# google-research/frame-interpolation

Hardware: AMD Instinct MI355X
Metric: interpolated frames/sec @1080p (higher is better)
Workload: dtype f32; 1 GPU; 1080p_2x2: 1920x1080 pair, align 64, block_shape [2, 2] -> 4 tile(s) of 960x576 in one batch, film_net published config, seeded synthetic weights, t=0.5; parallelism=1 independent GPU(s), weights RCCL-broadcast once, exec=direct launches, two lanes, lanes=1

## Files before the change

frame-interpolation_amd/csrc/conv_wino2d_impl.h:

```cpp
#pragma once
#include "conv_common.h"

enum { W2D_F_SQ = 128,
       W2D_F_XEPI = 8,
       W2D_DBG_TIME = 8192 };


template <bool SQ> struct W2dSlotTable { unsigned v[24 * 64]; };
template <bool SQ> constexpr W2dSlotTable<SQ> w2d_make_slot_table() {
  constexpr int QW = SQ ? 4 : 8, TH = SQ ? 16 : 8, HR = TH + 2, PW = 4 * QW + 2;
  constexpr int CO4 = (PW + 3) / 4, MO4 = 4 * CO4, RP4 = 4 * MO4 + (SQ ? 2 : 4);
  W2dSlotTable<SQ> t{};
  for (int sl = 0; sl < 24 * 64; ++sl) {
    const int r = sl / RP4, rem = sl % RP4, m = rem / MO4, rr = rem % MO4, c = rr / CO4, k = rr % CO4, px = 4 * k + m;
    const bool ok = r < HR && rem < 4 * MO4 && px < PW;
    t.v[sl] = ok ? ((unsigned)r << 24 | (unsigned)px << 8 | (unsigned)c << 4) : 0xFFFFFFFFu;
  }
  return t;
}
template <bool SQ> __device__ const W2dSlotTable<SQ> w2d_slot_table = w2d_make_slot_table<SQ>();

template <int BN, int FLAGS, int NS_ = 3>
__global__ __launch_bounds__(4 * (BN / 32) * 64, (BN == 32) ? 2 : 1) void conv_wino2d_kernel(ConvParams p) {
  constexpr bool SQ = (FLAGS & W2D_F_SQ) != 0;
  constexpr int QW = SQ ? 4 : 8, TH = SQ ? 16 : 8, HR = TH + 2, PXW = 4 * QW, PW = PXW + 2;
  static_assert(QW * (TH / 2) == 32, "32 units per tile");
  constexpr int NG = BN / 32, NW = 4 * NG;
  constexpr int CO4 = (PW + 3) / 4, MO4 = 4 * CO4, RP4 = 4 * MO4 + (SQ ? 2 : 4);
  constexpr int NREQ = 24;
  constexpr int STAGE4 = NREQ * 64;
  constexpr int NS = NS_;
  static_assert(NS == 2 || NS == 3, "stages");
  constexpr int IPW = NREQ / NW;
  static_assert(NREQ % NW == 0, "requests per wave");
  static_assert(HR * RP4 <= STAGE4, "stage size");
  constexpr bool XE = (FLAGS & W2D_F_XEPI) != 0;
  constexpr unsigned OOB = 0xFFFFFFFFu;

  extern __shared__ __attribute__((aligned(1024))) float smem[];

  const int t = threadIdx.x;
  const int lane = t & 63;
  const int wv = __builtin_amdgcn_readfirstlane(t >> 6);
  const int l31 = lane & 31, half = lane >> 5;
  const int mu = wv & 3, ng = wv >> 2;

  unsigned long long tm0 = 0, tm1 = 0, tm2 = 0, tmA = 0, tmB = 0, tmC = 0, tmW = 0, tmE1 = 0, tmE2 = 0, tmE3 = 0;
  unsigned long long rt0 = 0;
  if constexpr ((FLAGS & W2D_DBG_TIME) != 0) { rt0 = __builtin_amdgcn_s_memrealtime(); tm0 = __builtin_readcyclecounter(); }

  int aH = p.H, aW = p.W, aNB = p.NB, aCtot = p.Ctot, aKsplit = p.ksplit, aNseg = p.nseg, aUnused = p.unused_chain;
// ... 298 lines not shown
    for (int r = 0; r < 16; ++r) {
      const float m0 = acc[0][r], m1 = acc[1][r], m2 = acc[2][r], m3 = acc[3][r], m4 = acc[4][r], m5 = acc[5][r];
      const float s34 = m3 + m4, d34 = m3 - m4, d12 = m1 - m2, s12 = m1 + m2;
      o[0][r] = ((m0 + m1) + m2) + s34;
      o[1][r] = __builtin_fmaf(2.f, d34, d12);
      o[2][r] = __builtin_fmaf(4.f, s34, s12);
      o[3][r] = d12 + __builtin_fmaf(8.f, d34, m5);
    }
    bf4* const xb = reinterpret_cast<bf4*>(smem);
    constexpr int XB4 = NG * 4 * 256;
    static_assert(2 * XB4 <= NS * STAGE4, "exchange buffers");
    const int widx = (ng * 4 + mu) * 256 + l31 * 8;
    const int rng = t >> 8, run = (t >> 3) & 31, rcg = t & 7;
    const int ridx = rng * 1024 + run * 8 + (rcg ^ (run & 7));
    const int nrd = n0 + rng * 32 + rcg * 4;
    const bool rawsum = XE && ksp > 1;
    const bool has_pw = XE && p.pw_out != nullptr;
    float b0 = 0.f, b1 = 0.f, b2 = 0.f, b3 = 0.f;
    if (!rawsum) { const float* const bp = p.bias + nrd; b0 = bp[0]; b1 = bp[1]; b2 = bp[2]; b3 = bp[3]; }
    const int oy = y0 + 2 * (run / QW), ox = x0 + 4 * (run % QW);
    const int ostr = rawsum ? p.Cout : p.ostride;
    const float slope = (p.leaky && !rawsum) ? 0.2f : 1.f;
    const int dyo = 2 * (run / QW), dxo = 4 * (run % QW), nth = rng * 32 + rcg * 4;
    const int cpix = (img * p.H + y0) * p.W + x0;
    float* obase = p.out;
    if (rawsum) { asm volatile(""); obase = p.part + (size_t)blockIdx.z * p.M * p.Cout; }
    float* const ocorner = obase + ((long long)cpix * ostr + n0);
    float* const orow = ocorner + (__umul24(__umul24(dyo, p.W) + dxo, ostr) + nth);
    float* pool_base = nullptr;
    if (XE && p.pool_out) {
      asm volatile("");
      const int ppix = (img * (p.H >> 1) + (y0 >> 1)) * (p.W >> 1) + (x0 >> 1);
      pool_base = p.pool_out + ((long long)ppix * p.pool_ostride + n0) + (__umul24(__umul24(dyo >> 1, p.W >> 1) + (dxo >> 1), p.pool_ostride) + nth);
    }
    constexpr int PWS = 68;
    float* const pwt = smem + 2 * XB4 * 4;
    float* const pww = pwt + TH * PXW * PWS;
    if (has_pw && t < 256) pww[t] = (t & 3) < p.pw_cout ? p.pw_w[(t >> 2) * p.pw_cout + (t & 3)] : 0.f;
    bf4 k0 = {0.f, 0.f, 0.f, 0.f}, k1 = {0.f, 0.f, 0.f, 0.f};
    auto write_round = [&](int jx, bf4* xw) {
  #pragma unroll
      for (int g = 0; g < 4; ++g) {
        bf4 v;
        v[0] = o[jx][4 * g]; v[1] = o[jx][4 * g + 1]; v[2] = o[jx][4 * g + 2]; v[3] = o[jx][4 * g + 3];
        xw[widx + ((2 * g + half) ^ (l31 & 7))] = v;
      }
    };
  #pragma unroll
    for (int jx = 0; jx < 4; ++jx) {
      bf4* const xw = xb + (jx & 1) * XB4;
      write_round(jx, xw);
      __syncthreads();
      if constexpr ((FLAGS & W2D_DBG_TIME) != 0) { if (jx == 0) tmE2 = __builtin_readcyclecounter(); if (jx == 3) tmE3 = __builtin_readcyclecounter(); }
// ... 18 lines not shown
          if (jx & 1) {
            bf4 pv;
  #pragma unroll
            for (int c = 0; c < 4; ++c) pv[c] = (((k0[c] + r0[c]) + k1[c]) + r1[c]) * 0.25f;
            if (oy < p.H && ox + jx < p.W) *reinterpret_cast<bf4*>(pool_base + (size_t)(jx >> 1) * p.pool_ostride) = pv;
          } else {
            k0 = r0; k1 = r1;
          }
        }
      } else {
        float* const tr = pwt + ((2 * (run / QW)) * PXW + 4 * (run % QW) + jx) * PWS + rng * 32 + rcg * 4;
        *reinterpret_cast<bf4*>(tr) = r0;
        *reinterpret_cast<bf4*>(tr + PXW * PWS) = r1;
      }
    }
    if (has_pw) {
      __syncthreads();
      if (t < TH * PXW) {
        const int y = y0 + t / PXW, x = x0 + (t % PXW);
        float a[4] = {0.f, 0.f, 0.f, 0.f};
        const bf4* row = reinterpret_cast<const bf4*>(pwt + t * PWS);
        const bf4* wq = reinterpret_cast<const bf4*>(pww);
  #pragma unroll 4
        for (int c4 = 0; c4 < 16; ++c4) {
          const bf4 v = row[c4];
  #pragma unroll
          for (int k = 0; k < 4; ++k) {
            const bf4 w = wq[c4 * 4 + k];
  #pragma unroll
            for (int j = 0; j < 4; ++j) a[j] = __builtin_fmaf(v[k], w[j], a[j]);
          }
// ... 25 lines not shown
  if constexpr ((FLAGS & W2D_DBG_TIME) != 0) {
    const unsigned long long tm3 = __builtin_readcyclecounter();
    if (t == 0) {
      unsigned long long* o8 = reinterpret_cast<unsigned long long*>(p.part) + (size_t)(blockIdx.y * gridDim.x + blockIdx.x) * 16;
      o8[0] = tm0; o8[1] = tm1; o8[2] = tm2; o8[3] = tm3; o8[4] = tmA; o8[5] = tmB; o8[6] = tmC; o8[7] = tmW;
      o8[8] = rt0; o8[9] = __builtin_amdgcn_s_memrealtime();
      o8[10] = (unsigned long long)__builtin_amdgcn_s_getreg((31 << 11) | 4) | ((unsigned long long)__builtin_amdgcn_s_getreg((31 << 11) | 20) << 32);
      o8[11] = tmE1; o8[12] = tmE2; o8[13] = tmE3; o8[14] = tmK; o8[15] = tmT;
    }
  }
}

template <int BN, int FLAGS, int NS = 3>
hipError_t conv_wino2d_launch(const ConvParams& p, hipStream_t s) {
  if (!(FLAGS & W2D_F_XEPI) && (p.ksplit > 1 || p.pool_out || p.pw_out)) return hipErrorInvalidValue;
  const size_t lds = p.pw_out ? (size_t)2 * (BN / 32) * 16 * 1024 + 256 * 68 * 4 + 1024 : (size_t)NS * 24 * 1024;
  constexpr int NT = 4 * (BN / 32) * 64;
  if (p.ksize != 3 || p.Ctot % 16 || p.Cout % BN) return hipErrorInvalidValue;
  if (p.ksplit > 1 && (!p.part || (reinterpret_cast<uintptr_t>(p.part) & 15) || p.Cout % 4 || p.pool_out || p.pw_out || p.ksplit > p.Ctot / 16)) return hipErrorInvalidValue;
  if (p.pw_out) {
    if (BN != 64 || p.Cout != 64 || p.pool_out || p.pw_cout < 1 || p.pw_cout > 4) return hipErrorInvalidValue;
  } else if (p.ostride % 4 || (reinterpret_cast<uintptr_t>(p.out) & 15)) return hipErrorInvalidValue;
  if (p.pool_out && ((p.H | p.W) & 1 || p.pool_ostride % 4 || (reinterpret_cast<uintptr_t>(p.pool_out) & 15))) return hipErrorInvalidValue;
  {
    long long nimg = p.NB;
    for (int i = 0; i < p.nseg; ++i) nimg = std::max<long long>(nimg, (long long)p.seg[i].bmod);
    if ((nimg + 1) * p.H * p.W >= (1ll << 31)) return hipErrorInvalidValue;
  }
  if (p.W <= 0 || p.H <= 0 || p.W >= (1 << 20) || p.ostride >= (1 << 22) || p.pool_ostride >= (1 << 22) || p.Cout >= (1 << 22) ||
      (long long)8 * p.W * (p.ostride > p.Cout ? p.ostride : p.Cout) >= (1ll << 31)) return hipErrorInvalidValue;
  for (int i = 0; i < p.nseg; ++i)
    if ((long long)p.W * p.seg[i].stride * 4 >= (1ll << 24) || p.seg[i].C % 16 || p.seg[i].stride % 4 || p.seg[i].stride <= 0 || p.seg[i].stride >= (1 << 22) || p.seg[i].up || (reinterpret_cast<uintptr_t>(p.seg[i].ptr) & 15)) return hipErrorInvalidValue;
  constexpr bool SQ = (FLAGS & W2D_F_SQ) != 0;
  const int ntx = SQ ? (p.W + 15) / 16 : (p.W + 31) / 32, nty = SQ ? (p.H + 15) / 16 : (p.H + 7) / 8;
  const int ntiles = p.NB * ntx * nty;
  dim3 grid((unsigned)ntiles, p.Cout / BN, (unsigned)(p.ksplit > 1 ? p.ksplit : 1));
  ConvParams q = p;
  bool exact = true;
  q.mg_nby = conv_magic(grid.y, (unsigned long long)grid.x * grid.y, exact);
  q.mg_tpi = conv_magic((unsigned long long)ntx * nty, (unsigned long long)ntiles + 1, exact);
  q.mg_ntx = conv_magic(ntx, (unsigned long long)ntx * nty, exact);
  q.tl_ntx = ntx; q.tl_tpi = ntx * nty;
  if (!exact) return hipErrorInvalidValue;
  return conv_launch<conv_wino2d_kernel<BN, FLAGS, NS>>(grid, dim3(NT), lds, s, q, 144 * 1024);
}

template <int BN, int FLAGS, int NS = 3>
hipError_t conv_wino2d_launch_any(const ConvParams& p, hipStream_t s) {
  if (p.ksplit > 1 || p.pool_out || p.pw_out) return conv_wino2d_launch<BN, FLAGS | W2D_F_XEPI, NS>(p, s);
  return conv_wino2d_launch<BN, FLAGS, NS>(p, s);
}
```

frame-interpolation_amd/csrc/film_engine.cpp:

```cpp
#include "film_internal.h"

namespace film_internal {

thread_local std::string g_create_error;

int fail(film_t* h, int code, const char* fmt, ...) {
  char buf[1024];
  va_list ap;
  va_start(ap, fmt);
  vsnprintf(buf, sizeof buf, fmt, ap);
  va_end(ap);
  if (h) h->err = buf; else g_create_error = buf;
  return code;
}

int copy_out_string(film_t* h, const std::string& s, char* buf, int64_t cap, int64_t* needed) {
  if (needed) *needed = (int64_t)s.size() + 1;
  if (!buf || cap < (int64_t)s.size() + 1) {
    if (!buf && needed) return FILM_OK;
    return fail(h, FILM_ERR_INVALID, "buffer too small: need %lld bytes", (long long)s.size() + 1);
  }
  memcpy(buf, s.c_str(), s.size() + 1);
  return FILM_OK;
}
// ... 23 lines not shown
    {"max_batch", &film_t::opt_max_batch, NONNEG, false},
    {"host_overlap", &film_t::opt_host_overlap, BOOL, false},
    {"block_overlap_h", &film_t::opt_block_overlap_h, AS_IS, false, -1, 65535, "block_overlap_h: -1 (what the align padding of a tile holds) or 0 .. 65535 rows"},
    {"block_overlap_w", &film_t::opt_block_overlap_w, AS_IS, false, -1, 65535, "block_overlap_w: -1 (what the align padding of a tile holds) or 0 .. 65535 columns"},
    {"scene_cut", &film_t::opt_scene_cut, AS_IS, false, 0, 1000, "scene_cut: 0 (off) or 1 .. 1000 permille of the histogram distance"},
    {"tune_ms", &film_t::opt_tune_ms, NONNEG, false},
    {"splitk", &film_t::opt_splitk, BOOL, true},
    {"pack_groups", nullptr, AS_IS, false, 1, 4, "pack_groups: 1 .. 4"},
    {"fuse", &film_t::opt_fuse, LOW5, true},
    {"fold2x2", &film_t::opt_fold2x2, AS_IS, true, 0, 2, "fold2x2: 0, 1 or 2"},
    {"planar", &film_t::opt_planar, BOOL, true},
    {"winograd", &film_t::opt_wino, AS_IS, true, 0, 3, "winograd: 0, 1, 2 or 3", FAM_WINO, 2, 2,
     "winograd = 2 (F(2,3) kernel on every level) needs a library built with FILM_EXTRA_FAMILIES=1"},
    {"halo_all", &film_t::opt_halo_all, BOOL, true, 0, 0, nullptr, FAM_HALO, 1, 1, "halo_all needs a library built with FILM_EXTRA_FAMILIES=1"},
    {"lanes", &film_t::opt_lanes, AS_IS, true, 0, 3, "lanes: 0, 1, 2 or 3"},
    {"wino2d", &film_t::opt_wino2d, AS_IS, true, 0, 2, "wino2d: 0, 1 or 2"},
    {"w2d_small_px", &film_t::opt_w2d_small_px, AS_IS, true, 0, 1 << 30, "w2d_small_px: pixels per image, 0 = never"},
    {"w2d_min_px", &film_t::opt_w2d_min_px, AS_IS, true, 1, 1 << 30, "w2d_min_px: pixels per image"},
    {"w2d_splitk", &film_t::opt_w2d_splitk, AS_IS, true, 0, 16, "w2d_splitk: 0 (off), 1 (default rule) or 2..16 (A/B: the cap on levels of <= 1024 pixels)"},
    {"w2d_shape", &film_t::opt_w2d_shape, AS_IS, true, -1, W2D_SHAPES - 1, "w2d_shape: -1 (autotuned) or a Wino2dTile shape index"},
    {"fold4_shape", &film_t::opt_fold4_shape, AS_IS, true, -1, F4_4x32, "fold4_shape: -1 (autotuned) or a Fold4Tile shape index"},
    {"w43_shape", &film_t::opt_w43_shape, AS_IS, true, -1, 31, "w43_shape: -1 (autotuned) or a Wino43Tile shape index"},
    {"precision", &film_t::opt_precision, AS_IS, true, 0, 2, "precision: 0 (f32), 1 (bf16x6) or 2 (bf16x3)", FAM_SPLIT6, 1, 2,
     "precision %d (bf16 split modes) needs a library built with FILM_EXTRA_FAMILIES=1; this build runs fp32 MFMA only"},
};
constexpr bool option_rows_complete() {
  for (const OptionRow& o : kOptions)
    if ((o.lo < o.hi) != (o.refusal != nullptr) || ((o.family != FAM_BUF) != (o.family_refusal != nullptr))) return false;
  return true;
}
// ... 665 lines not shown
  fs.primed = true; fs.slot = slot; fs.plan_id = P0->id; fs.geo = tp;
  fs.hist_valid = scene_k > 0; fs.cut = cut ? 1 : 0;
  unprime.armed = false;
  return FILM_OK;
}

int film_get_tap(film_t* h, const char* name, float* dst, int64_t cap, int64_t dims[4]) {
  if (!h || !name) return FILM_ERR_INVALID;
  if (h->plan_only) return fail(h, FILM_ERR_NO_DEVICE, "plan-only handle has no device");
  Plan* P = h->last_plan;
  if (!P || !P->arena) return fail(h, FILM_ERR_STATE, "no forward has run yet");
  const int bi = P->find(name);
  if (bi < 0) return fail(h, FILM_ERR_NOTFOUND, "unknown tap '%s'", name);
  const Buffer& b = P->bufs[bi];
  for (const OpDesc& op : P->ops)
    if (op.kind == OP_CONV && op.pw_out.buf >= 0 && op.out.buf == bi)
      return fail(h, FILM_ERR_STATE, "tap '%s' is not materialised: the RGB head is fused into the layer that produces it "
                  "(film_set_option \"fuse\" without bit 16 keeps it)", name);
  if (dims) { dims[0] = b.N; dims[1] = b.H; dims[2] = b.W; dims[3] = b.C; }
  if (!dst) return FILM_OK;
  if (cap < b.size()) return fail(h, FILM_ERR_INVALID, "capacity %lld < %lld floats", (long long)cap, (long long)b.size());
  HIPCHK(h, hipSetDevice(h->device));
  HIPCHK(h, hipDeviceSynchronize());
  if (!b.planar) {
    HIPCHK(h, hipMemcpy(dst, P->arena + b.off, (size_t)b.size() * sizeof(float), hipMemcpyDeviceToHost));
    return FILM_OK;
  }
  std::vector<float> raw((size_t)b.size());
  HIPCHK(h, hipMemcpy(raw.data(), P->arena + b.off, raw.size() * sizeof(float), hipMemcpyDeviceToHost));
  const int64_t npix = (int64_t)b.N * b.H * b.W;
  const int pc[3] = {b.planar, b.planar, b.C - 2 * b.planar};
// ... 72 lines not shown
```

frame-interpolation_amd/csrc/film_exec.cpp:

```cpp
#include "film_internal.h"

namespace film_internal {
namespace {
inline const float* cptr(const float* base, const View& v) { return base + v.off; }
inline float* mptr(float* base, const View& v) { return base + v.off; }
}

hipError_t launch_op(const OpDesc& op, float* arena, const float* wts, hipStream_t s) {
  switch (op.kind) {
    case OP_CONV: {
      ConvParams p{};
      p.nseg = op.nseg;
      for (int i = 0; i < op.nseg; ++i) {
        p.seg[i].ptr = cptr(arena, op.seg[i].v);
        p.seg[i].stride = op.seg[i].v.stride;
        p.seg[i].C = op.seg[i].v.C;
        p.seg[i].boff = op.seg[i].boff; p.seg[i].bmod = op.seg[i].bmod; p.seg[i].up = op.seg[i].up;
      }
      p.ksize = op.ksize;
      p.w = wts + op.*kConvFamily[op.family].weights;
      p.bias = wts + op.b_off;
      p.out = mptr(arena, op.out); p.ostride = op.out.stride;
      p.NB = op.NB; p.H = op.H; p.W = op.W; p.Cout = op.Cout; p.Ctot = op.Ctot; p.leaky = op.leaky;
      p.M = op.NB * op.H * op.W;
      p.fold = op.fold; p.py = op.py; p.px = op.px; p.ftaps = op.ftaps;
      p.ksplit = op.ksplit; p.part = op.ksplit > 1 ? arena + op.part_off : nullptr;
      if (op.out2.buf >= 0) { p.pool_out = mptr(arena, op.out2); p.pool_ostride = op.out2.stride; }
      if (op.pw_out.buf >= 0) {
        p.pw_w = wts + op.w2_off; p.pw_bias = wts + op.b2_off; p.pw_out = mptr(arena, op.pw_out); p.pw_ostride = op.pw_out.stride; p.pw_cout = op.pw_cout;
      }
      for (int q = 0; q < 4; ++q) { p.tdy[q] = (signed char)op.tdy[q]; p.tdx[q] = (signed char)op.tdx[q]; p.fold_woff[q] = op.fold_woff[q]; }
      return film_launch_conv(p, op.tile, s);
    }
    case OP_FLOW_HEAD: {
      FlowHeadParams p{};
      p.in = cptr(arena, op.in); p.istride = op.in.stride; p.Cin = op.Ctot;
      p.w3 = wts + op.w_off; p.b3 = wts + op.b_off; p.w4 = wts + op.w2_off; p.b4 = wts + op.b2_off;
      p.out = mptr(arena, op.out); p.M = (int)op.n;
      if (op.out2.buf >= 0) { p.add = cptr(arena, op.in2); p.sum = mptr(arena, op.out2); }
      return film_launch_flow_head(p, s);
    }
    case OP_CONV_PW: {
// ... 36 lines not shown
        p.pack_b = cptr(arena, op.pack_b); p.pack_f = cptr(arena, op.pack_f);
      }
      return film_launch_warp(p, s);
    }
    case OP_PACK_FLOW: {
      PackFlowParams p{};
      p.bflow = cptr(arena, op.in); p.fflow = cptr(arena, op.in2);
      p.dst = mptr(arena, op.out); p.dstride = op.out.stride; p.npix = op.n;
      return film_launch_pack_flow(p, s);
    }
  }
  return hipErrorInvalidValue;
}

bool batch_splittable(const OpDesc& op, int nparts) {
  return op.kind == OP_CONV && op.nseg == 1 && op.seg[0].bmod == 0 && op.seg[0].boff == 0 && op.seg[0].up == 0 && op.ksplit <= 1 && op.fold == 0 &&
         op.NB >= nparts && op.NB % nparts == 0 && (op.out2.buf < 0 || (!(op.H & 1) && !(op.W & 1)));
}
OpDesc batch_part(const OpDesc& op, int part, int nparts) {
  OpDesc q = op;
  q.NB = op.NB / nparts;
  const int64_t px = (int64_t)part * q.NB * op.H * op.W;
  q.seg[0].v.off += px * op.seg[0].v.stride;
  q.out.off += px * op.out.stride;
  if (op.out2.buf >= 0) q.out2.off += (int64_t)part * q.NB * (op.H / 2) * (op.W / 2) * op.out2.stride;
  if (op.pw_out.buf >= 0) q.pw_out.off += px * op.pw_out.stride;
  return q;
}

hipError_t issue_lanes(film_t* h, Plan* P, hipStream_t main, bool capturing, const LanePipe* lp) {
  const size_t nops = P->ops.size();
// ... 100 lines not shown
```

frame-interpolation_amd/csrc/film_internal.h:

```cpp
#pragma once
#include <hip/hip_runtime.h>

#include <algorithm>
#include <atomic>
#include <cmath>
#include <cstdarg>
#include <cstdint>
#include <cstdio>
#include <cstdlib>
#include <cstring>
#include <functional>
#include <map>
#include <memory>
#include <sstream>
#include <string>
#include <thread>
#include <vector>

#include "../../include/film_hip.h"
#include "film_kernels.h"

namespace film_internal {


// ... 32 lines not shown
  ConvFamily family = FAM_BUF;
  int64_t b_off = 0;
  int64_t w2_off = 0, b2_off = 0;
  int ksplit = 1;
  int64_t part_off = 0;
  int fold = 0, py = 0, px = 0;
  int ftaps = 0; int tdy[4] = {0, 0, 0, 0}, tdx[4] = {0, 0, 0, 0};
  int64_t fold_woff[4] = {0, 0, 0, 0};
  int lane = 0;
  std::vector<int> xdeps;
  bool signal = false;
  View in, in2, out;
  View pack_b, pack_f;
  View img_in, img_out;
  View pw_out; int pw_cout = 0;
  View in3, out2;
  int NB = 0, H = 0, W = 0;
  float fscale = 1.f;
  int src_brot = 0, flow_brot = 0, misc_nb = 0;
  int64_t n = 0;
  double flops = 0;
  double bytes = 0;
};

struct LayerPack : ConvWeights {
  std::string name;
  int kh, kw, cin, cout;
  std::vector<int> perm;
  bool c3 = false;
  bool kmajor() const { return !c3 && cout % 32 == 0; }
// ... 92 lines not shown
  int opt_graph = 2;
  int opt_profile = 0, opt_autotune = 1;
  int opt_max_batch = 0;
  int opt_block_overlap_h = 0, opt_block_overlap_w = 0;
  int opt_scene_cut = 0;
  int opt_host_overlap = 1;
  hipEvent_t pipe_ev[2] = {nullptr, nullptr};
  int opt_splitk = 1;
  int opt_fuse = 31;
  int opt_planar = 1;
  int opt_fold2x2 = 1;
  int opt_wino = 1;
  int opt_halo_all = 0;
  int opt_tune_ms = 0;
  int opt_lanes = 1;
  hipStream_t stream2 = nullptr;
  int opt_precision = 0;
  int opt_wino2d = 1;
  int opt_w2d_min_px = 1536;
  int opt_w2d_small_px = 256;
  int opt_w2d_splitk = 1;
  int opt_w2d_shape = -1;
  int opt_fold4_shape = -1;
  int opt_w43_shape = -1;
  std::string profile_json;
  std::map<std::string, int> tune_cache;
  std::map<std::string, int> tune_import;
};

extern "C" int film_ensure_groups_(film_t* h, int n);
// ... 65 lines not shown
```

frame-interpolation_amd/csrc/film_kernels.h:

```cpp
#pragma once
#include <hip/hip_runtime.h>
#include <stdint.h>

#include <vector>

#include "../../include/film_hip.h"

#define FILM_MAX_SEG 4
#define FILM_BK 16

struct ConvSeg {
  const float* ptr;
  int stride;
  int C;
  int boff, bmod;
  int up;
};

struct ConvParams {
  ConvSeg seg[FILM_MAX_SEG];
  int nseg;
  int ksize;
  const float* w;
  const float* bias;
// ... 5 lines not shown
  int M;
  int fold, py, px, ftaps;
  signed char tdy[4], tdx[4];
  long long fold_woff[4];
  int ksplit;
  float* part;
  int unused_chain;
  unsigned mg_tpi, mg_ntx, mg_nby;
  int tl_ntx, tl_tpi;
  float* pool_out;
  int pool_ostride;
  const float* pw_w;
  const float* pw_bias;
  float* pw_out;
  int pw_ostride, pw_cout;
};

struct FlowHeadParams {
  const float* in;
  int istride;
  int Cin;
  const float* w3;
  const float* b3;
  const float* w4;
  const float* b4;
  float* out;
  int M;
  const float* add;
  float* sum;
};
// ... 238 lines not shown
```

frame-interpolation_amd/csrc/film_planner.cpp:

```cpp
#include "film_internal.h"

namespace film_internal {

const char* const kKindName[OP_KINDS] = {"conv_mfma", "flow_head", "conv_pw", "pool", "flow_up", "flow_add", "warp", "pack_flow"};

namespace {
struct ConvSite {
  const LayerPack* L;
  int H, W;
  int ctot;
  bool folded;
  bool any_up;
  bool out_16b;
  bool segs_16b;
  bool segs_c16;
  bool halo_row_24bit;
  bool fold4_rows_32bit;
  int64_t px() const { return (int64_t)H * W; }
};

ConvSite conv_site(const LayerPack& L, const std::vector<SegDesc>& segs, const View& out, int H, int W, bool folded) {
  ConvSite s{&L, H, W, 0, folded, false, out.off % 4 == 0 && out.stride % 4 == 0, true, true, true,
             (int64_t)16 * W * std::max(out.stride, L.cout) < (1ll << 31)};
  for (const SegDesc& g : segs) {
// ... 317 lines not shown
        SegDesc a = seg(view(feat[l], d ? i1 : i0, 0, fc[l]));
        SegDesc b = seg(coarsest ? view(feat[l], d ? i0 : i1, 0, fc[l]) : view(warped[l], d * B, 0, fc[l]));
        View o = cur;
        o.off += (int64_t)d * B * Hl * Wl * nf;
        conv(tg + ":d" + std::to_string(d), prefix + "/conv_0", {a, b}, o, B, Hl, Wl, true);
      }
    }
    int which = 0;
    for (int j = 1; j < nconv; ++j) {
      View nxt = scratch(fp[which ^ 1], nf);
      conv(tg, prefix + "/conv_" + std::to_string(j), {seg(cur)}, nxt, N2, Hl, Wl, true);
      cur = nxt; which ^= 1;
    }
    const int64_t M = (int64_t)N2 * Hl * Wl;
    const std::string l3 = prefix + "/conv_" + std::to_string(nconv), l4 = prefix + "/conv_" + std::to_string(nconv + 1);
    if ((nf / 2) % 32 == 0) {
      View hid = scratch(fp[2], nf / 2);
      conv(tg, l3, {seg(cur)}, hid, N2, Hl, Wl, true);
      conv_pw(tg, l4, hid, view(res[l], 0, 0, 2), M, false);
    } else {
      const LayerPack &L3 = layer(l3), &L4 = layer(l4);
      OpDesc op;
      op.kind = OP_FLOW_HEAD; op.tag = tg + ":" + l3 + "+conv_" + std::to_string(nconv + 1);
      op.in = cur; op.out = view(res[l], 0, 0, 2); op.n = M; op.Ctot = nf;
      op.w_off = L3.w_off; op.b_off = L3.b_off; op.w2_off = L4.w_off; op.b2_off = L4.b_off;
      op.flops = 2.0 * op.n * (nf * 16 + 16 * 2); op.bytes = 4.0 * op.n * (nf + 2);
      P->ops.push_back(op);
    }
    if (!coarsest && (h->opt_fuse & FUSE_FLOW_ADD)) {
      OpDesc& head = P->ops.back();
      head.tag += "+v=res+up";
      head.in2 = view(vup[l], 0, 0, 2); head.out2 = view(v[l], 0, 0, 2);
    } else if (!coarsest) {
      OpDesc ad;
      ad.kind = OP_FLOW_ADD; ad.tag = tg + ":v=res+up";
      ad.in = view(res[l], 0, 0, 2); ad.in2 = view(vup[l], 0, 0, 2); ad.out = view(v[l], 0, 0, 2);
      ad.n = M * 2; ad.bytes = 4.0 * ad.n * 3;
      P->ops.push_back(ad);
    }
    if (l >= 4) to_lane(first_op, 1);
  }

  void emit_align(int l) {
    const size_t first_op = P->ops.size();
    const std::string tg = "align_l" + std::to_string(l);
    const bool pair = P->bufs[aligned[l]].planar > 0 && !seq;
    const bool misc16 = (h->opt_fuse & FUSE_MISC16) && !seq;
    if (pair) {
      warp(tg + ":warp_feat01", view(feat[l], 0, 0, fc[l]), view(v[l], 0, 0, 2), aligned_part(aligned[l], 0, fc[l]), N2, HL(l), WL(l), 0.5f);
      P->ops.back().flow_brot = B;
    }
    for (int s = 0; s < 2; ++s) {
      View fl = view(v[l], (1 - s) * B, 0, 2);
      if (!pair)
        warp(tg + ":warp_feat" + std::to_string(s), view(feat[l], s ? i1 : i0, 0, fc[l]), fl,
// ... 180 lines not shown
    j.num("off", v.off); j.num("stride", v.stride); j.num("C", v.C);
    o << "}";
  }
};

void json_op(JsonObject& j, const OpDesc& op, const Plan& P) {
  const FamilyCodes fc = family_codes(op.family);
  j.str("kind", kKindName[op.kind]); j.str("tag", op.tag); j.num("NB", op.NB); j.num("H", op.H); j.num("W", op.W);
  j.num("ksize", op.ksize); j.num("leaky", op.leaky); j.num("Cout", op.Cout); j.num("Ctot", op.Ctot); j.num("tile", op.tile);
  j.num("w_off", op.w_off); j.num("b_off", op.b_off); j.num("wf4_off", op.wf4_off);
  j.num("wh_off", op.wh_off); j.num("halo", fc.halo); j.num("ws_off", op.ws_off); j.num("split", fc.split);
  j.num("ww_off", op.ww_off); j.num("wx_off", op.wx_off); j.num("wfx_off", op.wfx_off); j.num("w43_off", op.w43_off); j.num("w2d_off", op.w2d_off);
  j.num("wino", fc.wino); j.num("fold", op.fold); j.num("ksplit", op.ksplit);
  j.num("py", op.py); j.num("px", op.px); j.num("ftaps", op.ftaps); j.ints("tdy", op.tdy, 4); j.ints("tdx", op.tdx, 4);
  j.ints("fold_woff", op.fold_woff, 4); j.num("lane", op.lane); j.ints("xdeps", op.xdeps.data(), op.xdeps.size());
  j.num("w2_off", op.w2_off); j.num("b2_off", op.b2_off); j.num("c3", fc.c3);
  j.num("fscale", op.fscale); j.num("src_brot", op.src_brot); j.num("flow_brot", op.flow_brot); j.num("misc_nb", op.misc_nb); j.num("n", op.n);
  j.num("flops", op.flops); j.num("bytes", op.bytes);
  j.view("in", op.in, P); j.view("in2", op.in2, P); j.view("in3", op.in3, P); j.view("out2", op.out2, P); j.view("pw_out", op.pw_out, P); j.num("pw_cout", op.pw_cout);
  j.view("img_in", op.img_in, P); j.view("img_out", op.img_out, P); j.view("pack_b", op.pack_b, P); j.view("pack_f", op.pack_f, P); j.view("out", op.out, P);
  j.objects("segs", op.seg, op.nseg, [&](JsonObject& s, const SegDesc& g) {
    s.view("v", g.v, P); s.num("boff", g.boff); s.num("bmod", g.bmod); s.num("up", g.up);
  });
}
}

std::string plan_json(film_t* h, const Plan& P) {
  std::ostringstream o;
  JsonObject j{o};
  j.num("B", P.B); j.num("H", P.H); j.num("W", P.W);
  if (P.slot >= 0) { j.str("kind", "stream"); j.num("tiles", P.tiles); j.num("slot", P.slot); j.num("n_extract", P.n_extract); }
// ... 16 lines not shown
```

frame-interpolation_amd/csrc/film_tune.cpp:

```cpp
#include "film_internal.h"

namespace film_internal {
namespace {
std::vector<int> both_maps(ConvFamily f, const std::vector<int>& shapes) {
  std::vector<int> out;
  for (int sh : shapes) { out.push_back(conv_tile(f, sh, false)); out.push_back(conv_tile(f, sh, true)); }
  return out;
}

std::string conv_signature(const OpDesc& op) {
  std::ostringstream o;
  const FamilyCodes fc = family_codes(op.family);
  o << op.NB << 'x' << op.H << 'x' << op.W << ':' << op.Cout << ':' << op.ksize << ':' << op.out.stride << ':' << fc.c3 << ':' << fc.halo << ':' << fc.split << ':' << fc.wino << ':' << op.fold << ':' << op.ksplit << ':' << (op.out2.buf >= 0) << ':' << op.pw_cout;
  for (int i = 0; i < op.nseg; ++i)
    o << '|' << op.seg[i].v.C << ',' << op.seg[i].v.stride << ',' << op.seg[i].up << ',' << op.seg[i].bmod;
  return o.str();
}
}

std::vector<int> tile_candidates(const OpDesc& op) {
  if (op.Cout % 128 == 0) return both_maps(FAM_BUF, {TILE_128x128, TILE_256x128, TILE_256x64, TILE_128x64, TILE_64x64});
  if (op.Cout % 64 == 0) return both_maps(FAM_BUF, {TILE_256x64, TILE_128x64, TILE_64x64, TILE_256x32, TILE_128x32});
  return both_maps(FAM_BUF, {TILE_256x32, TILE_128x32});
}

std::vector<int> c3_candidates(const OpDesc&) { return {conv_tile(FAM_C3, TILE_C3_DIRECT, false)}; }

std::vector<int> halo_candidates(const OpDesc& op) {
// ... 18 lines not shown
              W43_Q16_4x64_T21_P2, W43_Q16_4x64_T12_P2, W43_Q16_4x32_T11_P2, W43_Q16_4x64_N1_P2, W43_Q16_4x32_T11_BG,
              W43_Q8_8x64_T21_P2, W43_Q8_8x64_T12_P2, W43_Q8_8x64_N1_P2, W43_Q8_8x32_T11_BG, W43_Q8_8x32_T11_P2};
  else
    shapes = {W43_4x32_T11, W43_Q16_4x32_T11, W43_Q16_4x32_T11_P2, W43_Q16_4x32_T11_BG, W43_Q8_8x32_T11_BG, W43_Q8_8x32_T11_P2};
  std::vector<int> keep;
  for (int sh : shapes) {
    if (!film_w43_shape_built(sh)) continue;
    if (pool && (sh == W43_4x64_T21 || sh == W43_4x64_T12 || sh == W43_4x32_T11)) continue;
    keep.push_back(sh);
  }
  return both_maps(FAM_W43, keep);
}

std::vector<int> wino2d_candidates(const OpDesc& op) {
  const int H = op.H, W = op.W;
  const bool pw = op.pw_out.buf >= 0;
  const int64_t pad_r = (int64_t)((W + 31) / 32) * ((H + 7) / 8), pad_s = (int64_t)((W + 15) / 16) * ((H + 15) / 16);
  const bool sq = pad_s <= pad_r;
  std::vector<int> shapes;
  if (pw || op.Cout % 64 == 0) { shapes.push_back(W2D_8x64); if (sq) shapes.push_back(W2D_16x64); }
  if (!pw) {
    shapes.push_back(W2D_8x32); shapes.push_back(W2D_8x32_S2);
    if (sq) { shapes.push_back(W2D_16x32); shapes.push_back(W2D_16x32_S2); }
  }
  return both_maps(FAM_W2D, shapes);
}

std::vector<int> fold4_candidates(const OpDesc& op) {
  return both_maps(FAM_FOLD4, op.Cout % 64 == 0 ? std::vector<int>{F4_4x64, F4_4x32} : std::vector<int>{F4_4x32});
}

std::vector<int> foldx3_candidates(const OpDesc& op) {
  return both_maps(FAM_FOLDX3, op.Cout % 128 == 0 ? std::vector<int>{FX3_4x64, FX3_8x64, FX3_4x128} : std::vector<int>{FX3_4x64, FX3_8x64});
}

// ... 130 lines not shown
```

Baseline: 29.99 frames/s.

## Fuse flow-head 1x1 convs and residual add into Winograd 3x3 conv epilogue

Adds a W2D_F_HEAD variant of the Winograd 2D conv kernel. Its epilogue runs the flow head's hidden 1x1 conv (nf to nf/2 with leaky ReLU), the final 1x1 conv to 2 channels and the optional residual flow add, all from LDS. The planner folds the two 1x1 layers into the preceding 3x3 conv on large 32-filter levels by default, and on more levels with other option values. This removes the write and re-read of the hidden activation and the extra launches. In exchange the kernel needs more LDS and its tile choices are restricted, and the fused ops can no longer be split by batch.

After: 30.22 frames/s (median of 6 runs). No clear change (+0.8%).

```diff
diff --git a/frame-interpolation_amd/csrc/conv_wino2d_impl.h b/frame-interpolation_amd/csrc/conv_wino2d_impl.h
--- a/frame-interpolation_amd/csrc/conv_wino2d_impl.h
+++ b/frame-interpolation_amd/csrc/conv_wino2d_impl.h
@@ -3,6 +3,7 @@
 
 enum { W2D_F_SQ = 128,
        W2D_F_XEPI = 8,
+       W2D_F_HEAD = 16,
        W2D_DBG_TIME = 8192 };
 
 
@@ -35,6 +36,7 @@
   static_assert(NREQ % NW == 0, "requests per wave");
   static_assert(HR * RP4 <= STAGE4, "stage size");
   constexpr bool XE = (FLAGS & W2D_F_XEPI) != 0;
+  constexpr bool FH = XE && (FLAGS & W2D_F_HEAD) != 0;
   constexpr unsigned OOB = 0xFFFFFFFFu;
 
   extern __shared__ __attribute__((aligned(1024))) float smem[];
@@ -363,8 +365,8 @@
     const int rng = t >> 8, run = (t >> 3) & 31, rcg = t & 7;
     const int ridx = rng * 1024 + run * 8 + (rcg ^ (run & 7));
     const int nrd = n0 + rng * 32 + rcg * 4;
-    const bool rawsum = XE && ksp > 1;
-    const bool has_pw = XE && p.pw_out != nullptr;
+    const bool rawsum = XE && !FH && ksp > 1;
+    const bool has_pw = FH || (XE && p.pw_out != nullptr);
     float b0 = 0.f, b1 = 0.f, b2 = 0.f, b3 = 0.f;
     if (!rawsum) { const float* const bp = p.bias + nrd; b0 = bp[0]; b1 = bp[1]; b2 = bp[2]; b3 = bp[3]; }
     const int oy = y0 + 2 * (run / QW), ox = x0 + 4 * (run % QW);
@@ -377,15 +379,21 @@
     float* const ocorner = obase + ((long long)cpix * ostr + n0);
     float* const orow = ocorner + (__umul24(__umul24(dyo, p.W) + dxo, ostr) + nth);
     float* pool_base = nullptr;
-    if (XE && p.pool_out) {
+    if (XE && !FH && p.pool_out) {
       asm volatile("");
       const int ppix = (img * (p.H >> 1) + (y0 >> 1)) * (p.W >> 1) + (x0 >> 1);
       pool_base = p.pool_out + ((long long)ppix * p.pool_ostride + n0) + (__umul24(__umul24(dyo >> 1, p.W >> 1) + (dxo >> 1), p.pool_ostride) + nth);
     }
-    constexpr int PWS = 68;
+    constexpr int PWS = BN + 4;
+    constexpr int HC = BN / 2;
     float* const pwt = smem + 2 * XB4 * 4;
     float* const pww = pwt + TH * PXW * PWS;
-    if (has_pw && t < 256) pww[t] = (t & 3) < p.pw_cout ? p.pw_w[(t >> 2) * p.pw_cout + (t & 3)] : 0.f;
+    if constexpr (FH) {
+      for (int i = t; i < BN * HC; i += NW * 64) pww[i] = p.hid_kmajor ? p.hid_w[(i % HC) * BN + i / HC] : p.hid_w[i];
+      if (t < HC) pww[BN * HC + t] = p.hid_bias[t];
+      if (t < 2 * HC) pww[BN * HC + HC + t] = p.pw_w[t];
+      if (t < 2) pww[BN * HC + 3 * HC + t] = p.pw_bias[t];
+    } else if (has_pw && t < 256) pww[t] = (t & 3) < p.pw_cout ? p.pw_w[(t >> 2) * p.pw_cout + (t & 3)] : 0.f;
     bf4 k0 = {0.f, 0.f, 0.f, 0.f}, k1 = {0.f, 0.f, 0.f, 0.f};
     auto write_round = [&](int jx, bf4* xw) {
   #pragma unroll
@@ -434,7 +442,50 @@
         *reinterpret_cast<bf4*>(tr + PXW * PWS) = r1;
       }
     }
-    if (has_pw) {
+    if constexpr (FH) {
+      __syncthreads();
+      if (t < TH * PXW) {
+        const int y = y0 + t / PXW, x = x0 + (t % PXW);
+        float hv[HC];
+  #pragma unroll
+        for (int o = 0; o < HC; ++o) hv[o] = 0.f;
+        const bf4* row = reinterpret_cast<const bf4*>(pwt + t * PWS);
+        const bf4* w3 = reinterpret_cast<const bf4*>(pww);
+  #pragma unroll 2
+        for (int c4 = 0; c4 < BN / 4; ++c4) {
+          const bf4 v = row[c4];
+  #pragma unroll
+          for (int k = 0; k < 4; ++k) {
+  #pragma unroll
+            for (int o4 = 0; o4 < HC / 4; ++o4) {
+              const bf4 w = w3[(c4 * 4 + k) * (HC / 4) + o4];
+  #pragma unroll
+              for (int j = 0; j < 4; ++j) hv[o4 * 4 + j] = __builtin_fmaf(v[k], w[j], hv[o4 * 4 + j]);
+            }
+          }
+        }
+        const float* const b3s = pww + BN * HC;
+        const float* const w4s = b3s + HC;
+        float o0 = 0.f, o1 = 0.f;
+  #pragma unroll
+        for (int o = 0; o < HC; ++o) {
+          const float hh = leaky02(hv[o] + b3s[o]);
+          o0 = __builtin_fmaf(hh, w4s[o * 2], o0);
+          o1 = __builtin_fmaf(hh, w4s[o * 2 + 1], o1);
+        }
+        if (y < p.H && x < p.W) {
+          const size_t m = ((size_t)img * p.H + y) * p.W + x;
+          const float r0 = o0 + w4s[2 * HC], r1 = o1 + w4s[2 * HC + 1];
+          float* const rd = p.pw_out + m * 2;
+          rd[0] = r0; rd[1] = r1;
+          if (p.pw_add != nullptr) {
+            const float* const ua = p.pw_add + m * 2;
+            float* const sd = p.pw_sum + m * 2;
+            sd[0] = r0 + ua[0]; sd[1] = r1 + ua[1];
+          }
+        }
+      }
+    } else if (has_pw) {
       __syncthreads();
       if (t < TH * PXW) {
         const int y = y0 + t / PXW, x = x0 + (t % PXW);
@@ -490,11 +541,18 @@
 template <int BN, int FLAGS, int NS = 3>
 hipError_t conv_wino2d_launch(const ConvParams& p, hipStream_t s) {
   if (!(FLAGS & W2D_F_XEPI) && (p.ksplit > 1 || p.pool_out || p.pw_out)) return hipErrorInvalidValue;
-  const size_t lds = p.pw_out ? (size_t)2 * (BN / 32) * 16 * 1024 + 256 * 68 * 4 + 1024 : (size_t)NS * 24 * 1024;
+  constexpr bool FH = (FLAGS & W2D_F_HEAD) != 0;
+  if (FH != (p.hid_w != nullptr)) return hipErrorInvalidValue;
+  const size_t lds_pw = FH ? (size_t)2 * (BN / 32) * 16 * 1024 + 256 * (BN + 4) * 4 + (BN * (BN / 2) + 3 * (BN / 2) + 2 + 2) * 4
+                           : (size_t)2 * (BN / 32) * 16 * 1024 + 256 * 68 * 4 + 1024;
+  const size_t lds = p.pw_out ? std::max(lds_pw, (size_t)NS * 24 * 1024) : (size_t)NS * 24 * 1024;
   constexpr int NT = 4 * (BN / 32) * 64;
   if (p.ksize != 3 || p.Ctot % 16 || p.Cout % BN) return hipErrorInvalidValue;
   if (p.ksplit > 1 && (!p.part || (reinterpret_cast<uintptr_t>(p.part) & 15) || p.Cout % 4 || p.pool_out || p.pw_out || p.ksplit > p.Ctot / 16)) return hipErrorInvalidValue;
-  if (p.pw_out) {
+  if (FH) {
+    if (p.Cout != BN || !p.pw_out || !p.pw_w || !p.pw_bias || !p.hid_bias || p.pw_cout != 2 || p.pw_ostride != 2 || p.pool_out || p.ksplit > 1 ||
+        (p.pw_add != nullptr) != (p.pw_sum != nullptr)) return hipErrorInvalidValue;
+  } else if (p.pw_out) {
     if (BN != 64 || p.Cout != 64 || p.pool_out || p.pw_cout < 1 || p.pw_cout > 4) return hipErrorInvalidValue;
   } else if (p.ostride % 4 || (reinterpret_cast<uintptr_t>(p.out) & 15)) return hipErrorInvalidValue;
   if (p.pool_out && ((p.H | p.W) & 1 || p.pool_ostride % 4 || (reinterpret_cast<uintptr_t>(p.pool_out) & 15))) return hipErrorInvalidValue;
@@ -523,6 +581,7 @@
 
 template <int BN, int FLAGS, int NS = 3>
 hipError_t conv_wino2d_launch_any(const ConvParams& p, hipStream_t s) {
+  if (p.hid_w) return conv_wino2d_launch<BN, FLAGS | W2D_F_XEPI | W2D_F_HEAD, NS>(p, s);
   if (p.ksplit > 1 || p.pool_out || p.pw_out) return conv_wino2d_launch<BN, FLAGS | W2D_F_XEPI, NS>(p, s);
   return conv_wino2d_launch<BN, FLAGS, NS>(p, s);
 }
diff --git a/frame-interpolation_amd/csrc/film_engine.cpp b/frame-interpolation_amd/csrc/film_engine.cpp
--- a/frame-interpolation_amd/csrc/film_engine.cpp
+++ b/frame-interpolation_amd/csrc/film_engine.cpp
@@ -61,6 +61,7 @@
      "winograd = 2 (F(2,3) kernel on every level) needs a library built with FILM_EXTRA_FAMILIES=1"},
     {"halo_all", &film_t::opt_halo_all, BOOL, true, 0, 0, nullptr, FAM_HALO, 1, 1, "halo_all needs a library built with FILM_EXTRA_FAMILIES=1"},
     {"lanes", &film_t::opt_lanes, AS_IS, true, 0, 3, "lanes: 0, 1, 2 or 3"},
+    {"flow_head_fuse", &film_t::opt_flow_head_fuse, AS_IS, true, 0, 3, "flow_head_fuse: 0 (never), 1 (32-filter levels of >= 100 000 pixels), 2 (every eligible level) or 3 (1 and the 64-filter levels)"},
     {"wino2d", &film_t::opt_wino2d, AS_IS, true, 0, 2, "wino2d: 0, 1 or 2"},
     {"w2d_small_px", &film_t::opt_w2d_small_px, AS_IS, true, 0, 1 << 30, "w2d_small_px: pixels per image, 0 = never"},
     {"w2d_min_px", &film_t::opt_w2d_min_px, AS_IS, true, 1, 1 << 30, "w2d_min_px: pixels per image"},
@@ -756,7 +757,7 @@
   if (bi < 0) return fail(h, FILM_ERR_NOTFOUND, "unknown tap '%s'", name);
   const Buffer& b = P->bufs[bi];
   for (const OpDesc& op : P->ops)
-    if (op.kind == OP_CONV && op.pw_out.buf >= 0 && op.out.buf == bi)
+    if (op.kind == OP_CONV && op.pw_out.buf >= 0 && op.w3_off < 0 && op.out.buf == bi)
       return fail(h, FILM_ERR_STATE, "tap '%s' is not materialised: the RGB head is fused into the layer that produces it "
                   "(film_set_option \"fuse\" without bit 16 keeps it)", name);
   if (dims) { dims[0] = b.N; dims[1] = b.H; dims[2] = b.W; dims[3] = b.C; }
diff --git a/frame-interpolation_amd/csrc/film_exec.cpp b/frame-interpolation_amd/csrc/film_exec.cpp
--- a/frame-interpolation_amd/csrc/film_exec.cpp
+++ b/frame-interpolation_amd/csrc/film_exec.cpp
@@ -25,7 +25,10 @@
       p.M = op.NB * op.H * op.W;
       p.fold = op.fold; p.py = op.py; p.px = op.px; p.ftaps = op.ftaps;
       p.ksplit = op.ksplit; p.part = op.ksplit > 1 ? arena + op.part_off : nullptr;
-      if (op.out2.buf >= 0) { p.pool_out = mptr(arena, op.out2); p.pool_ostride = op.out2.stride; }
+      if (op.w3_off >= 0) {
+        p.hid_w = wts + op.w3_off; p.hid_bias = wts + op.b3_off; p.hid_kmajor = op.hid_kmajor;
+        if (op.out2.buf >= 0) { p.pw_add = cptr(arena, op.in3); p.pw_sum = mptr(arena, op.out2); }
+      } else if (op.out2.buf >= 0) { p.pool_out = mptr(arena, op.out2); p.pool_ostride = op.out2.stride; }
       if (op.pw_out.buf >= 0) {
         p.pw_w = wts + op.w2_off; p.pw_bias = wts + op.b2_off; p.pw_out = mptr(arena, op.pw_out); p.pw_ostride = op.pw_out.stride; p.pw_cout = op.pw_cout;
       }
@@ -92,7 +95,7 @@
 }
 
 bool batch_splittable(const OpDesc& op, int nparts) {
-  return op.kind == OP_CONV && op.nseg == 1 && op.seg[0].bmod == 0 && op.seg[0].boff == 0 && op.seg[0].up == 0 && op.ksplit <= 1 && op.fold == 0 &&
+  return op.kind == OP_CONV && op.w3_off < 0 && op.nseg == 1 && op.seg[0].bmod == 0 && op.seg[0].boff == 0 && op.seg[0].up == 0 && op.ksplit <= 1 && op.fold == 0 &&
          op.NB >= nparts && op.NB % nparts == 0 && (op.out2.buf < 0 || (!(op.H & 1) && !(op.W & 1)));
 }
 OpDesc batch_part(const OpDesc& op, int part, int nparts) {
diff --git a/frame-interpolation_amd/csrc/film_internal.h b/frame-interpolation_amd/csrc/film_internal.h
--- a/frame-interpolation_amd/csrc/film_internal.h
+++ b/frame-interpolation_amd/csrc/film_internal.h
@@ -70,6 +70,7 @@
   View pack_b, pack_f;
   View img_in, img_out;
   View pw_out; int pw_cout = 0;
+  int64_t w3_off = -1, b3_off = -1; int hid_kmajor = 0;
   View in3, out2;
   int NB = 0, H = 0, W = 0;
   float fscale = 1.f;
@@ -192,6 +193,7 @@
   int opt_halo_all = 0;
   int opt_tune_ms = 0;
   int opt_lanes = 1;
+  int opt_flow_head_fuse = 1;
   hipStream_t stream2 = nullptr;
   int opt_precision = 0;
   int opt_wino2d = 1;
diff --git a/frame-interpolation_amd/csrc/film_kernels.h b/frame-interpolation_amd/csrc/film_kernels.h
--- a/frame-interpolation_amd/csrc/film_kernels.h
+++ b/frame-interpolation_amd/csrc/film_kernels.h
@@ -43,6 +43,11 @@
   const float* pw_bias;
   float* pw_out;
   int pw_ostride, pw_cout;
+  const float* hid_w;
+  const float* hid_bias;
+  int hid_kmajor;
+  const float* pw_add;
+  float* pw_sum;
 };
 
 struct FlowHeadParams {
diff --git a/frame-interpolation_amd/csrc/film_planner.cpp b/frame-interpolation_amd/csrc/film_planner.cpp
--- a/frame-interpolation_amd/csrc/film_planner.cpp
+++ b/frame-interpolation_amd/csrc/film_planner.cpp
@@ -355,7 +355,8 @@
     }
     const int64_t M = (int64_t)N2 * Hl * Wl;
     const std::string l3 = prefix + "/conv_" + std::to_string(nconv), l4 = prefix + "/conv_" + std::to_string(nconv + 1);
-    if ((nf / 2) % 32 == 0) {
+    if (fuse_flow_head(l, nf, l3, l4, M)) {
+    } else if ((nf / 2) % 32 == 0) {
       View hid = scratch(fp[2], nf / 2);
       conv(tg, l3, {seg(cur)}, hid, N2, Hl, Wl, true);
       conv_pw(tg, l4, hid, view(res[l], 0, 0, 2), M, false);
@@ -371,7 +372,7 @@
     if (!coarsest && (h->opt_fuse & FUSE_FLOW_ADD)) {
       OpDesc& head = P->ops.back();
       head.tag += "+v=res+up";
-      head.in2 = view(vup[l], 0, 0, 2); head.out2 = view(v[l], 0, 0, 2);
+      (head.kind == OP_CONV ? head.in3 : head.in2) = view(vup[l], 0, 0, 2); head.out2 = view(v[l], 0, 0, 2);
     } else if (!coarsest) {
       OpDesc ad;
       ad.kind = OP_FLOW_ADD; ad.tag = tg + ":v=res+up";
@@ -380,6 +381,26 @@
       P->ops.push_back(ad);
     }
     if (l >= 4) to_lane(first_op, 1);
+  }
+
+  bool fuse_flow_head(int l, int nf, const std::string& l3, const std::string& l4, int64_t M) {
+    if (!h->opt_flow_head_fuse || P->ops.empty()) return false;
+    if (h->opt_flow_head_fuse != 2 && (int64_t)HL(l) * WL(l) < 100000) return false;
+    if (h->opt_flow_head_fuse == 1 && nf != 32) return false;
+    OpDesc& cv = P->ops.back();
+    const LayerPack &L3 = layer(l3), &L4 = layer(l4);
+    if (cv.kind != OP_CONV || cv.family != FAM_W2D || cv.ksize != 3 || cv.Cout != nf || (nf != 32 && nf != 64) || cv.ksplit > 1 || cv.out2.buf >= 0 ||
+        cv.pw_out.buf >= 0 || L3.kh != 1 || L3.kw != 1 || L3.cin != nf || L3.ctot() != nf || L3.cout != nf / 2 || L4.kh != 1 || L4.cin != nf / 2 || L4.cout != 2 ||
+        L4.kmajor())
+      return false;
+    cv.tag += "+conv_" + l3.substr(l3.rfind('_') + 1) + "+conv_" + l4.substr(l4.rfind('_') + 1);
+    cv.w3_off = L3.w_off; cv.b3_off = L3.b_off; cv.hid_kmajor = L3.kmajor() ? 1 : 0;
+    cv.w2_off = L4.w_off; cv.b2_off = L4.b_off;
+    cv.pw_out = view(res[l], 0, 0, 2); cv.pw_cout = 2;
+    cv.tile = conv_tile(FAM_W2D, nf == 64 ? W2D_8x64 : W2D_8x32, true);
+    cv.flops += 2.0 * M * (nf * (nf / 2) + (nf / 2) * 2);
+    cv.bytes += nf / 2 == 16 ? 4.0 * M * (nf + 2) : 4.0 * M * (nf + nf / 2) + 4.0 * M * (nf / 2 + 2);
+    return true;
   }
 
   void emit_align(int l) {
@@ -590,7 +611,7 @@
   j.num("wino", fc.wino); j.num("fold", op.fold); j.num("ksplit", op.ksplit);
   j.num("py", op.py); j.num("px", op.px); j.num("ftaps", op.ftaps); j.ints("tdy", op.tdy, 4); j.ints("tdx", op.tdx, 4);
   j.ints("fold_woff", op.fold_woff, 4); j.num("lane", op.lane); j.ints("xdeps", op.xdeps.data(), op.xdeps.size());
-  j.num("w2_off", op.w2_off); j.num("b2_off", op.b2_off); j.num("c3", fc.c3);
+  j.num("w2_off", op.w2_off); j.num("b2_off", op.b2_off); j.num("w3_off", op.w3_off); j.num("b3_off", op.b3_off); j.num("hid_kmajor", op.hid_kmajor); j.num("c3", fc.c3);
   j.num("fscale", op.fscale); j.num("src_brot", op.src_brot); j.num("flow_brot", op.flow_brot); j.num("misc_nb", op.misc_nb); j.num("n", op.n);
   j.num("flops", op.flops); j.num("bytes", op.bytes);
   j.view("in", op.in, P); j.view("in2", op.in2, P); j.view("in3", op.in3, P); j.view("out2", op.out2, P); j.view("pw_out", op.pw_out, P); j.num("pw_cout", op.pw_cout);
diff --git a/frame-interpolation_amd/csrc/film_tune.cpp b/frame-interpolation_amd/csrc/film_tune.cpp
--- a/frame-interpolation_amd/csrc/film_tune.cpp
+++ b/frame-interpolation_amd/csrc/film_tune.cpp
@@ -12,6 +12,7 @@
   std::ostringstream o;
   const FamilyCodes fc = family_codes(op.family);
   o << op.NB << 'x' << op.H << 'x' << op.W << ':' << op.Cout << ':' << op.ksize << ':' << op.out.stride << ':' << fc.c3 << ':' << fc.halo << ':' << fc.split << ':' << fc.wino << ':' << op.fold << ':' << op.ksplit << ':' << (op.out2.buf >= 0) << ':' << op.pw_cout;
+  if (op.w3_off >= 0) o << ":head" << op.hid_kmajor;
   for (int i = 0; i < op.nseg; ++i)
     o << '|' << op.seg[i].v.C << ',' << op.seg[i].v.stride << ',' << op.seg[i].up << ',' << op.seg[i].bmod;
   return o.str();
@@ -60,11 +61,11 @@
 
 std::vector<int> wino2d_candidates(const OpDesc& op) {
   const int H = op.H, W = op.W;
-  const bool pw = op.pw_out.buf >= 0;
+  const bool pw = op.pw_out.buf >= 0 && !(op.w3_off >= 0 && op.Cout == 32);
   const int64_t pad_r = (int64_t)((W + 31) / 32) * ((H + 7) / 8), pad_s = (int64_t)((W + 15) / 16) * ((H + 15) / 16);
   const bool sq = pad_s <= pad_r;
   std::vector<int> shapes;
-  if (pw || op.Cout % 64 == 0) { shapes.push_back(W2D_8x64); if (sq) shapes.push_back(W2D_16x64); }
+  if (pw || (op.Cout % 64 == 0 && op.w3_off < 0)) { shapes.push_back(W2D_8x64); if (sq) shapes.push_back(W2D_16x64); }
   if (!pw) {
     shapes.push_back(W2D_8x32); shapes.push_back(W2D_8x32_S2);
     if (sq) { shapes.push_back(W2D_16x32); shapes.push_back(W2D_16x32_S2); }
```
